# UbiquityRobotics/fiducials

Hardware: NVIDIA H100
Metric: frames/sec 1920x1080 (detect+pose) (higher is better)
Workload: dtype u8/i32 (threshold, contours), f32/f64 (sub-pixel, pose, map)

## Files before the change

### fiducials_b200/csrc/fid_api.cu

```cuda
#include <cuda.h>
#include <cuda_runtime.h>
#include <stdio.h>
#include <stdlib.h>
#include <string.h>

#include <algorithm>
#include <cmath>
#include <vector>

#include "../../include/fiducials_b200.h"
#include "kernels_contour.cuh"
#include "kernels_threshold.cuh"
#include "start_prune_table.h"
#include "kernels_threshold_mma.cuh"
#include "kernels_marker.cuh"
#include "kernels_aruco3.cuh"
#include "params_host.h"

using namespace fid;

#define CK(call)                                                                                       \
    do {                                                                                               \
        cudaError_t e_ = (call);                                                                       \
        if (e_ != cudaSuccess) {                                                                       \
// ... 226 lines not shown
template <class T>
static int halloc(T** p, size_t count) {
    if (cudaMallocHost((void**)p, count * sizeof(T)) != cudaSuccess) {
        cudaGetLastError();
        return FID_ERR_NO_MEMORY;
    }
    return FID_OK;
}

static FrameGeom make_geom(const fid_detector* h, int W, int H, size_t row_stride, size_t frame_stride) {
    FrameGeom g;
    g.W = W;
    g.H = H;
    g.gray_pitch = (W + 31) / 32 * 32;
    g.bgr_row_stride = row_stride;
    g.bgr_frame_stride = frame_stride;
    g.gray_frame_stride = (size_t)g.gray_pitch * H;
    g.halo_tpr = halo_tiles_x(W);
    g.halo_tiles_y = (H + FID_HALO_T - 1) / FID_HALO_T;
    g.halo_scale_stride = halo_plane_words(W, H);
    g.halo_frame_stride = g.halo_scale_stride * h->P.n_scales;
    g.magic_tpr = (uint32_t)((0x100000000ull + (uint64_t)g.halo_tpr - 1) / (uint64_t)g.halo_tpr);
    g.magic_tiles_y = (uint32_t)((0x100000000ull + (uint64_t)g.halo_tiles_y - 1) / (uint64_t)g.halo_tiles_y);
    return g;
}

static int upload_dictionary(fid_detector* h) {
    std::vector<unsigned long long> words;
    pack_dictionary(h->P, &words);
    CK(cudaMemcpy(h->d_dict, words.data(), words.size() * sizeof(unsigned long long), cudaMemcpyHostToDevice));
    return FID_OK;
}

static size_t group_smem(int max_raw) { return (size_t)max_raw * 6 * sizeof(int) + (((size_t)max_raw + 15) & ~(size_t)15) + GROUP_CLOSE_SMEM_WORDS * sizeof(uint32_t); }
static size_t ident_smem(const DevParams& P, int warps) { return (size_t)P.n_markers * 4 * 8 + (size_t)warps * 256 * 4 + (size_t)warps * FID_MAX_WARP_SIDE_SQ; }

typedef CUresult (*EncodeTiledFn)(CUtensorMap*, CUtensorMapDataType, cuuint32_t, void*, const cuuint64_t*, const cuuint64_t*, const cuuint32_t*, const cuuint32_t*, CUtensorMapInterleave,
                                  CUtensorMapSwizzle, CUtensorMapL2promotion, CUtensorMapFloatOOBfill);
static EncodeTiledFn encode_tiled_fn() {
    static EncodeTiledFn fn = nullptr;
    static bool tried = false;
    if (!tried) {
        tried = true;
        void* p = nullptr;
        cudaDriverEntryPointQueryResult q;
        if (cudaGetDriverEntryPoint("cuTensorMapEncodeTiled", &p, cudaEnableDefault, &q) == cudaSuccess && q == cudaDriverEntryPointSuccess) fn = (EncodeTiledFn)p;
        cudaGetLastError();
    }
    return fn;
}
static bool make_bgr_tensor_map(CUtensorMap* tm, const uint8_t* src, int W, int H, int nf, size_t row_stride, size_t frame_stride) {
    EncodeTiledFn fn = encode_tiled_fn();
    if (!fn || (W & 3) || (row_stride & 15) || (frame_stride & 15) || (reinterpret_cast<uintptr_t>(src) & 15) || 3 * W / 4 < TM_BOXW || H < TM_BOXH) return false;
    const cuuint64_t gdim[3] = {(cuuint64_t)(3 * W / 4), (cuuint64_t)H, (cuuint64_t)nf};
    const cuuint64_t gstr[2] = {(cuuint64_t)row_stride, (cuuint64_t)frame_stride};
    const cuuint32_t box[3] = {TM_BOXW, TM_BOXH, 1};
    const cuuint32_t estr[3] = {1, 1, 1};
    return fn(tm, CU_TENSOR_MAP_DATA_TYPE_UINT32, 3, const_cast<uint8_t*>(src), gdim, gstr, box, estr, CU_TENSOR_MAP_INTERLEAVE_NONE, CU_TENSOR_MAP_SWIZZLE_NONE,
              CU_TENSOR_MAP_L2_PROMOTION_L2_128B, CU_TENSOR_MAP_FLOAT_OOB_FILL_NONE) == CUDA_SUCCESS;
}

static int r_max_of(const DevParams& P) {
    int r = 1;
    for (int i = 0; i < P.n_scales; i++) r = std::max(r, P.win[i] / 2);
    return r;
}

static int configure_kernels(fid_detector* h) {
    CK(cudaFuncSetAttribute(k_threshold<true>, cudaFuncAttributeMaxDynamicSharedMemorySize, (int)thresh_smem_bytes(THR_FAST_R)));
    CK(cudaFuncSetAttribute(k_threshold<false>, cudaFuncAttributeMaxDynamicSharedMemorySize, (int)thresh_smem_bytes(FID_MAX_WIN_RADIUS)));
    CK(cudaFuncSetAttribute(k_threshold<true, true>, cudaFuncAttributeMaxDynamicSharedMemorySize, (int)thresh_smem_bytes(THR_FAST_R)));
    CK(cudaFuncSetAttribute(k_threshold<false, true>, cudaFuncAttributeMaxDynamicSharedMemorySize, (int)thresh_smem_bytes(FID_MAX_WIN_RADIUS)));
    CK(cudaFuncSetAttribute(k_threshold_mma<false>, cudaFuncAttributeMaxDynamicSharedMemorySize, (int)TM_SMEM_BYTES));
    CK(cudaFuncSetAttribute(k_threshold_mma<true>, cudaFuncAttributeMaxDynamicSharedMemorySize, (int)TM_SMEM_BYTES));
    for (auto k : {k_sort_group<false>, k_sort_group<true>}) CK(cudaFuncSetAttribute(k, cudaFuncAttributeMaxDynamicSharedMemorySize, (int)group_smem(FID_GROUP_MAX_RAW)));
    for (auto k : {k_identify_retry<false>, k_identify_retry<true>, k_identify_retry<false, true>, k_identify_retry<true, true>, k_identify_retry<false, false, true>,
                   k_identify_retry<true, false, true>, k_identify_retry<false, true, true>, k_identify_retry<true, true, true>})
        CK(cudaFuncSetAttribute(k, cudaFuncAttributeMaxDynamicSharedMemorySize, (int)(kMaxDictMarkers * 4 * 8 + IDENT_WARPS * 256 * 4 + IDENT_WARPS * FID_MAX_WARP_SIDE_SQ)));
    for (auto k : {k_identify_first<false>, k_identify_first<true>, k_identify_first<false, true>, k_identify_first<true, true>, k_identify_first<false, false, true>,
                   k_identify_first<true, false, true>, k_identify_first<false, true, true>, k_identify_first<true, true, true>})
        CK(cudaFuncSetAttribute(k, cudaFuncAttributeMaxDynamicSharedMemorySize, (int)(kMaxDictMarkers * 4 * 8 + IDENT0_WARPS * 256 * 4 + IDENT0_WARPS * FID_MAX_WARP_SIDE_SQ)));
    return FID_OK;
}

static int alloc_slot(fid_detector* h, Slot& s) {
    const size_t F = h->max_batch;
    const int W = h->max_w, H = h->max_h;
    const size_t wpr = (W + 31) / 32, pitch = wpr * 32;
    const int S = FID_MAX_SCALES;
    int rc;
#define A(expr)                  \
    if ((rc = (expr)) != FID_OK) return rc;
    A(dalloc(&s.d_bgr, F * (size_t)W * H * 3));
    A(dalloc(&s.d_gray, F * pitch * H));
    A(dalloc(&s.d_halo, F * (size_t)S * halo_plane_words(W, H)));
    A(dalloc(&s.d_starts, (size_t)h->max_starts));
    A(dalloc(&s.d_chains, (size_t)h->max_chains));
    A(dalloc(&s.d_segs, (size_t)h->max_segs));
    A(dalloc(&s.d_queue[0], (size_t)h->max_queue));
    A(dalloc(&s.d_queue[1], (size_t)h->max_queue));
    A(dalloc(&s.d_points, (size_t)h->max_points));
    A(dalloc(&s.d_counters, 1));
    const size_t R = F * h->max_raw;
    A(dalloc(&s.d_raw, R));
    A(dalloc(&s.d_nraw, F));
    A(dalloc(&s.fs.quads_tmp, R));
    A(dalloc(&s.fs.per_tmp, R));
    A(dalloc(&s.fs.quads, R));
    A(dalloc(&s.fs.per, R));
    A(dalloc(&s.fs.close_bits, R * h->close_wpr));
    A(dalloc(&s.fs.group_id, R));
    A(dalloc(&s.fs.group_members, R));
    A(dalloc(&s.fs.next_in_group, R));
    A(dalloc(&s.fs.group_head, R));
    A(dalloc(&s.fs.group_tail, R));
    A(dalloc(&s.fs.close_count, R));
    A(dalloc(&s.fs.close_idx, R));
    A(dalloc(&s.fs.close_off, R));
    A(dalloc(&s.fs.selected, R));
    A(dalloc(&s.fs.sel_idx, R));
    A(dalloc(&s.fs.raw_of_sorted, R));
    A(dalloc(&s.d_nsel, F));
    A(dalloc(&s.d_nrawc, F));
    A(dalloc(&s.d_cand_id, F * h->max_sel));
    A(dalloc(&s.d_cand_corners, F * h->max_sel * 8));
    A(dalloc(&s.d_cand_raw, F * h->max_sel));
    A(dalloc(&s.d_first_list, F * h->max_sel));
    A(dalloc(&s.d_retry_list, F * h->max_sel));
    const size_t M = F * h->max_markers;
    A(dalloc(&s.d_out_count, F));
    A(dalloc(&s.d_out_ids, M));
    A(dalloc(&s.d_out_corners, M * 8));
    A(dalloc(&s.d_out_tf, M));
    A(halloc(&s.h_out_count, F));
    A(halloc(&s.h_out_ids, M));
    A(halloc(&s.h_out_corners, M * 8));
    A(halloc(&s.h_out_tf, M));
    A(halloc(&s.h_counters, 1));
    A(halloc(&s.h_nsel, F));
    A(halloc(&s.h_nrawc, F));
#undef A
    for (int i = 0; i <= ST_COUNT; i++) CK(cudaEventCreate(&s.ev[i]));
    for (int i = 0; i <= N_WALK_ROUNDS; i++) CK(cudaEventCreate(&s.ev_round[i]));
    CK(cudaEventCreateWithFlags(&s.done, cudaEventDisableTiming));
    CK(cudaEventCreateWithFlags(&s.copied, cudaEventDisableTiming));
// ... 670 lines not shown
    }
    CK(cudaEventRecord(s.ev[ST_APPROX], st));
    {
        ApproxArgs a{};
        a.chains = s.d_chains;
        a.points = s.d_points;
        a.counters = s.d_counters;
        a.raw = s.d_raw;
        a.n_raw = s.d_nraw;
        a.counters_rw = s.d_counters;
        a.max_chains = h->max_chains;
        a.max_raw = h->max_raw;
        a.W = W;
        a.H = H;
        a.poly_accuracy_rate = P.poly_accuracy_rate;
        a.min_corner_dist_rate = P.min_corner_dist_rate;
        launch_prio(k_approx_warp, dim3(h->sm_count * 8), dim3(APPROX_THREADS), 0, st, 3, a);
        launches++;
        launch_prio(k_approx, dim3(h->sm_count * 4), dim3(APPROX_THREADS), 0, st, 3, a);
        launches++;
    }
    CK(cudaEventRecord(s.ev[ST_GROUP], st));
    if (stop_after == ST_APPROX) return FID_OK;
    auto group = [&](int marker_size) {
        GroupArgs a{};
        a.raw = s.d_raw;
        a.n_raw = s.d_nraw;
        a.fs = s.fs;
        a.n_sel = s.d_nsel;
        a.n_raw_clamped = s.d_nrawc;
        a.max_raw = h->max_raw;
        a.close_wpr = h->close_wpr;
        a.max_sel = h->max_sel;
        a.marker_size = marker_size;
        a.border_bits = P.marker_border_bits;
        a.min_marker_dist_rate = (float)P.min_marker_dist_rate;
        a.min_group_dist = (float)P.min_group_dist;
        a.W = W;
        a.H = H;
        a.min_dist_to_border = P.min_dist_to_border;
        a.counters = s.d_counters;
        a.first_list = s.d_first_list;
        static const int group_prof = getenv("FID_GROUP_PROF") ? atoi(getenv("FID_GROUP_PROF")) : 0;
        a.prof = group_prof;
        launch_prio(inv ? k_sort_group<true> : k_sort_group<false>, dim3(nf), dim3(GROUP_THREADS), group_smem(h->max_raw), st, 4, a);
        launches++;
    };
    auto identify = [&](const DevParams& Pd, const unsigned long long* dict) {
        IdentifyArgs a{};
        a.src = d_bgr;
        a.row_stride = g.bgr_row_stride;
        a.frame_stride = g.bgr_frame_stride;
        a.enc = h->enc;
        a.W = g.W;
        a.H = g.H;
        a.fs = s.fs;
        a.n_sel = s.d_nsel;
        a.max_raw = h->max_raw;
        a.max_sel = h->max_sel;
        a.P = Pd;
        a.dict = dict;
        a.cand_id = s.d_cand_id;
        a.cand_corners = s.d_cand_corners;
        a.cand_raw = s.d_cand_raw;
        a.first_list = s.d_first_list;
        a.retry_list = s.d_retry_list;
        a.counters = s.d_counters;
        if (a3) a.pyr = A3Pyramid{s.d_gray, g.gray_frame_stride, s.d_a3_pyr, s.d_raw, ag};
        if (inv) {
            static void (*const first[2][2])(const IdentifyArgs) = {{k_identify_first<false, false, true>, k_identify_first<false, true, true>},
                                                                    {k_identify_first<true, false, true>, k_identify_first<true, true, true>}};
            static void (*const retry[2][2])(const IdentifyArgs) = {{k_identify_retry<false, false, true>, k_identify_retry<false, true, true>},
                                                                    {k_identify_retry<true, false, true>, k_identify_retry<true, true, true>}};
            if (conf) a.cand_conf = s.d_cand_conf;
            launch_prio(first[a3][conf], dim3(h->sm_count * 4), dim3(IDENT0_WARPS * 32), ident_smem(Pd, IDENT0_WARPS), st, 4, a);
            launch_prio(retry[a3][conf], dim3(h->sm_count * 2), dim3(IDENT_WARPS * 32), ident_smem(Pd, IDENT_WARPS), st, 4, a);
        } else if (conf) {
            a.cand_conf = s.d_cand_conf;
// ... 1621 lines not shown
```

### fiducials_b200/csrc/kernels_marker.cuh

```cuda
#pragma once
#include <cuda_runtime.h>

#include "../../include/fiducials_b200.h"
#include "aruco3.cuh"
#include "board_pnp.cuh"
#include "candidate_tree.cuh"
#include "charuco.cuh"
#include "common.cuh"
#include "contour_refine.cuh"
#include "diamond.cuh"
#include "identify.cuh"
#include "ippe.cuh"
#include "marker_refine.cuh"
#include "pnp.cuh"
#include "quad_group.cuh"
#include "subpix.cuh"

namespace fid {


struct FrameScratch {
    QuadF* quads_tmp;
    float* per_tmp;
    QuadF* quads;
    float* per;
    uint32_t* close_bits;
    int* group_id;
    int* group_members;
    int* next_in_group;
    int* group_head;
    int* group_tail;
    int* close_count;
    int* close_idx;
    int* close_off;
    uint8_t* selected;
    int* sel_idx;
    int* raw_of_sorted;
};

struct GroupArgs {
    const RawQuad* raw;
    const unsigned int* n_raw;
    FrameScratch fs;
    int* n_sel;
    int* n_raw_clamped;
    int max_raw, close_wpr, max_sel;
    int marker_size, border_bits;
    float min_marker_dist_rate, min_group_dist;
    int W, H, min_dist_to_border;
    Counters* counters;
    uint32_t* first_list;
    int prof;
};

struct WarpLanes {
    __device__ int lane() const { return threadIdx.x & 31; }
    __device__ int count() const { return 32; }
    __device__ void sync() const { __syncwarp(); }
    __device__ long long sum(long long v) const {
#pragma unroll
        for (int d = 16; d > 0; d >>= 1) v += __shfl_xor_sync(0xffffffffu, v, d);
        return v;
    }
    __device__ int min_i(int v) const {
#pragma unroll
        for (int d = 16; d > 0; d >>= 1) {
            const int o = __shfl_xor_sync(0xffffffffu, v, d);
            v = o < v ? o : v;
        }
        return v;
    }
    __device__ unsigned long long or_u64(unsigned long long v) const {
#pragma unroll
        for (int d = 16; d > 0; d >>= 1) v |= __shfl_xor_sync(0xffffffffu, v, d);
        return v;
    }
    __device__ void hist_add(int* h, int bin) const { atomicAdd(h + bin, 1); }
    __device__ uint32_t ballot(bool p) const { return __ballot_sync(0xffffffffu, p); }
    __device__ int shfl_i(int v, int src) const { return __shfl_sync(0xffffffffu, v, src); }
    __device__ int atomic_add(int* p, int v) const { return atomicAdd(p, v); }
};

#define GROUP_THREADS 1024
#define FID_GROUP_MAX_RAW 4096
#define GROUP_CLOSE_SMEM_WORDS 12288

template <bool INV = false>
__global__ void __launch_bounds__(GROUP_THREADS) k_sort_group(const GroupArgs a) {
    const int f = blockIdx.x;
    const int tid = threadIdx.x;
    int n = (int)a.n_raw[f];
    n = n < a.max_raw ? n : a.max_raw;
    const size_t fo = (size_t)f * a.max_raw;
    const RawQuad* raw = a.raw + fo;
    QuadF* qt = a.fs.quads_tmp + fo;
    float* pt = a.fs.per_tmp + fo;
    QuadF* qs = a.fs.quads + fo;
    float* ps = a.fs.per + fo;
    long long t_[7] = {0, 0, 0, 0, 0, 0, 0};
#define GROUP_TICK(k) if (a.prof && tid == 0 && f == 0) t_[k] = clock64()
    GROUP_TICK(0);
    if (tid == 0) a.n_raw_clamped[f] = n;
    extern __shared__ int sm_group[];
    float* s_f0 = reinterpret_cast<float*>(sm_group);
    float* s_f1 = s_f0 + a.max_raw;
    float* s_f2 = s_f1 + a.max_raw;
    for (int i = tid; i < n; i += GROUP_THREADS) {
        const QuadF q = quad_clockwise(raw[i]);
        qt[i] = q;
        const float p = quad_perimeter(q);
        pt[i] = p;
        s_f0[i] = p;
    }
    __syncthreads();
    for (int i = tid; i < n; i += GROUP_THREADS) {
        const float pi = s_f0[i];
        const uint32_t hi = raw[i].order_hi, lo = raw[i].order_lo;
        int rank = 0;
        for (int j = 0; j < n; j++) {
            const float pj = s_f0[j];
            const bool before = pj > pi || (pj == pi && (raw[j].order_hi < hi || (raw[j].order_hi == hi && raw[j].order_lo < lo)));
            rank += before ? 1 : 0;
        }
        qs[rank] = qt[i];
        ps[rank] = pi;
        a.fs.raw_of_sorted[fo + rank] = i;
    }
    __syncthreads();
    QuadF* s_quads = reinterpret_cast<QuadF*>(s_f2 + a.max_raw);
    const bool quads_in_smem = (size_t)n * sizeof(QuadF) <= (size_t)3 * a.max_raw * sizeof(int);
    for (int i = tid; i < n; i += GROUP_THREADS) {
        const QuadF q = qs[i];
        s_f0[i] = (q.x[0] + q.x[1] + q.x[2] + q.x[3]) * 0.25f;
        s_f1[i] = (q.y[0] + q.y[1] + q.y[2] + q.y[3]) * 0.25f;
        s_f2[i] = ps[i] * a.min_marker_dist_rate;
        if (quads_in_smem) s_quads[i] = q;
    }
    __syncthreads();
    GROUP_TICK(1);
    __shared__ uint32_t row_any[(FID_GROUP_MAX_RAW + 31) / 32], grouped[(FID_GROUP_MAX_RAW + 31) / 32];
    int* sm_group_id = sm_group;
    int* sm_members = sm_group + a.max_raw;
    int* sm_next = sm_group + 3 * a.max_raw;
    int* sm_head = sm_group + 4 * a.max_raw;
    int* sm_tail = sm_group + 5 * a.max_raw;
    uint8_t* sm_selected = reinterpret_cast<uint8_t*>(sm_group + 6 * a.max_raw);
    __shared__ int s_warp_cnt[GROUP_THREADS / 32];
    __shared__ int s_base;
    for (int i = tid; i < (FID_GROUP_MAX_RAW + 31) / 32; i += GROUP_THREADS) row_any[i] = 0;
    __syncthreads();
    const int wpr = (n + 31) >> 5;
    uint32_t* sm_close = reinterpret_cast<uint32_t*>(sm_selected + ((a.max_raw + 15) & ~15));
    const bool close_in_smem = n * wpr <= GROUP_CLOSE_SMEM_WORDS;
    uint32_t* cb = close_in_smem ? sm_close : a.fs.close_bits + fo * a.close_wpr;
    const int cb_pitch = close_in_smem ? wpr : a.close_wpr;
    {
        const int warp = tid >> 5, lane = tid & 31;
        for (int u = warp; u < n * wpr; u += GROUP_THREADS / 32) {
            const int i = u / wpr, w = u - i * wpr;
            const int j0 = w << 5;
            uint32_t bits = 0;
            if (j0 + 31 > i) {
                const int j = j0 + lane;
                bool close = false;
                if (j > i && j < n) {
                    const float thr = s_f2[j];
                    const float dx = s_f0[i] - s_f0[j], dy = s_f1[i] - s_f1[j];
                    const float cd2 = dx * dx + dy * dy;
                    const float lim = thr * 1.01f + 1.0f;
                    if (cd2 <= lim * lim) close = (quads_in_smem ? quad_avg_distance(s_quads[i], s_quads[j]) : quad_avg_distance(qs[i], qs[j])) < thr;
                }
                bits = __ballot_sync(0xffffffffu, close);
            }
            if (lane == 0) {
                cb[(size_t)i * cb_pitch + w] = bits;
                if (bits) atomicOr(&row_any[i >> 5], 1u << (i & 31));
            }
        }
    }
    __syncthreads();
    GROUP_TICK(2);
    __shared__ int s_n_groups, s_total_close, s_members_used;
    __shared__ uint32_t s_row[2][FID_GROUP_MAX_RAW / 32], s_rowmask[2][4];
    if (tid < 32) {
        struct RowPtr {
            const uint32_t* p;
            __device__ uint32_t operator()(int w) const { return p[w]; }
        };
        const int lane = tid;
        int n_groups = 0;
        if (lane == 0) group_pairs_init(n, sm_selected, sm_group_id, sm_next, a.fs.close_count + fo, grouped);
        __syncwarp();
        auto next_row = [&](int i) {
            while (i < n && !((row_any[i >> 5] >> (i & 31)) & 1u)) i++;
            return i;
        };
        if (close_in_smem) {
            if (lane == 0)
                for (int i = next_row(0); i < n; i = next_row(i + 1))
                    group_pairs_row(n, i, RowPtr{sm_close + (size_t)i * wpr}, nullptr, &n_groups, sm_selected, sm_group_id, sm_next, sm_head, sm_tail, grouped);
        } else {
            uint32_t v[3][4];
            int rows[3];
            rows[0] = next_row(0);
            rows[1] = rows[0] < n ? next_row(rows[0] + 1) : n;
            rows[2] = rows[1] < n ? next_row(rows[1] + 1) : n;
#pragma unroll
            for (int r = 0; r < 3; r++)
#pragma unroll
                for (int k = 0; k < 4; k++) v[r][k] = (rows[r] < n && lane + 32 * k < wpr) ? cb[(size_t)rows[r] * cb_pitch + lane + 32 * k] : 0u;
            int buf = 0;
            while (rows[0] < n) {
                const int i = rows[0];
#pragma unroll
                for (int k = 0; k < 4; k++) {
                    if (lane + 32 * k < wpr) s_row[buf][lane + 32 * k] = v[0][k];
                    const uint32_t nz = __ballot_sync(0xffffffffu, v[0][k] != 0u);
                    if (lane == 0) s_rowmask[buf][k] = nz;
                }
                __syncwarp();
                const int inext = rows[2] < n ? next_row(rows[2] + 1) : n;
#pragma unroll
                for (int k = 0; k < 4; k++) {
                    v[0][k] = v[1][k];
                    v[1][k] = v[2][k];
                    v[2][k] = (inext < n && lane + 32 * k < wpr) ? cb[(size_t)inext * cb_pitch + lane + 32 * k] : 0u;
                }
                rows[0] = rows[1];
                rows[1] = rows[2];
                rows[2] = inext;
                if (lane == 0) group_pairs_row(n, i, RowPtr{s_row[buf]}, s_rowmask[buf], &n_groups, sm_selected, sm_group_id, sm_next, sm_head, sm_tail, grouped);
                __syncwarp();
                buf ^= 1;
// ... 70 lines not shown
    int* cand_id;
    float* cand_corners;
    int* cand_raw;
    const uint32_t* first_list;
    uint32_t* retry_list;
    Counters* counters;
    A3Pyramid pyr;
    float* cand_conf;
};

#define IDENT_WARPS 8
#define IDENT0_WARPS 4

__device__ __forceinline__ void identify_write(const IdentifyArgs& a, size_t fo, size_t o, int id, int rot, int used) {
    a.cand_id[o] = id;
    a.cand_raw[o] = a.fs.raw_of_sorted[fo + used];
    const QuadF use = a.fs.quads[fo + used];
    for (int c = 0; c < 4; c++) {
        a.cand_corners[o * 8 + 2 * c] = use.x[(c + 4 - rot) & 3];
        a.cand_corners[o * 8 + 2 * c + 1] = use.y[(c + 4 - rot) & 3];
    }
}

template <bool PYR, bool CONF, bool INV>
__device__ __forceinline__ IdentifyResult identify_attempt(const IdentifyArgs& a, const WarpLanes& L, int f, int level, const QuadF& quad, const unsigned long long* dict,
                                                           uint8_t* img, int* hist) {
    if constexpr (PYR) {
        const float s = a3_level_scale(a.pyr.g, level);
        QuadF q;
        for (int c = 0; c < 4; c++) {
            q.x[c] = quad.x[c] * s;
            q.y[c] = quad.y[c] * s;
        }
        return identify_candidate<CONF, INV>(L, a.pyr.plane(f, level), a.pyr.g.lv[level].W, a.pyr.g.lv[level].H, q, a.P, dict, img, hist);
    } else {
        const FrameImg gray{a.src + (size_t)f * a.frame_stride, a.row_stride, a.enc};
        return identify_candidate<CONF, INV>(L, gray, a.W, a.H, quad, a.P, dict, img, hist);
    }
}
template <bool PYR>
__device__ __forceinline__ int identify_level(const IdentifyArgs& a, size_t fo, int si) {
    if constexpr (PYR)
        return a3_level_for(a.pyr.g, a.pyr.raw[fo + a.fs.raw_of_sorted[fo + si]].n_contour);
    else
        return 0;
}

template <bool PYR, bool CONF = false, bool INV = false>
__global__ void __launch_bounds__(IDENT0_WARPS * 32) k_identify_first(const IdentifyArgs a) {
    extern __shared__ unsigned long long sm_dict[];
    const unsigned int n_first = a.counters->n_first;
    if (blockIdx.x * IDENT0_WARPS >= n_first) return;
    const int n_words = a.P.n_markers * 4;
    for (int i = threadIdx.x; i < n_words; i += blockDim.x) sm_dict[i] = __ldg(a.dict + i);
    const int warp = threadIdx.x >> 5, lane = threadIdx.x & 31;
    int* hist = reinterpret_cast<int*>(sm_dict + n_words) + warp * 256;
    uint8_t* img = reinterpret_cast<uint8_t*>(reinterpret_cast<int*>(sm_dict + n_words) + IDENT0_WARPS * 256) + warp * (FID_MAX_WARP_SIDE_SQ);
    __syncthreads();
    WarpLanes L;
    for (unsigned int i = blockIdx.x * IDENT0_WARPS + warp; i < n_first; i += gridDim.x * IDENT0_WARPS) {
        const uint32_t rec = a.first_list[i];
        const int f = (int)(rec >> 16), k = (int)(rec & 0xFFFFu);
        const size_t fo = (size_t)f * a.max_raw, o = (size_t)f * a.max_sel + k;
        const int si = a.fs.sel_idx[fo + k];
        const IdentifyResult r = identify_attempt<PYR, CONF, INV>(a, L, f, identify_level<PYR>(a, fo, si), a.fs.quads[fo + si], sm_dict, img, hist);
        __syncwarp();
        if (lane == 0) {
            if (r.id >= 0) {
                identify_write(a, fo, o, r.id, r.rotation, si);
                if constexpr (CONF) a.cand_conf[o] = marker_confidence(hist, a.P, sm_dict[r.id * 4 + r.rotation]);
            } else if (a.fs.close_count[fo + si] > 0) {
                a.cand_id[o] = -2;
                a.retry_list[atomicAdd(&a.counters->n_retry, 1u)] = rec;
            } else {
                a.cand_id[o] = -1;
            }
        }
        if constexpr (CONF) __syncwarp();
    }
}

template <bool PYR, bool CONF = false, bool INV = false>
__global__ void __launch_bounds__(IDENT_WARPS * 32) k_identify_retry(const IdentifyArgs a) {
    extern __shared__ unsigned long long sm_dict[];
    __shared__ int s_best;
    __shared__ int s_id[IDENT_WARPS], s_rot[IDENT_WARPS], s_att[IDENT_WARPS];
    const unsigned int n_retry = a.counters->n_retry;
    if (blockIdx.x >= n_retry) return;
    const int n_words = a.P.n_markers * 4;
    for (int i = threadIdx.x; i < n_words; i += blockDim.x) sm_dict[i] = __ldg(a.dict + i);
    const int warp = threadIdx.x >> 5, lane = threadIdx.x & 31;
    int* hist = reinterpret_cast<int*>(sm_dict + n_words) + warp * 256;
    uint8_t* img = reinterpret_cast<uint8_t*>(reinterpret_cast<int*>(sm_dict + n_words) + IDENT_WARPS * 256) + warp * (FID_MAX_WARP_SIDE_SQ);
    WarpLanes L;
    for (unsigned int i = blockIdx.x; i < n_retry; i += gridDim.x) {
        const uint32_t rec = a.retry_list[i];
        const int f = (int)(rec >> 16), k = (int)(rec & 0xFFFFu);
        const size_t fo = (size_t)f * a.max_raw, o = (size_t)f * a.max_sel + k;
        __syncthreads();
        if (threadIdx.x == 0) s_best = 0x7fffffff;
        if (lane == 0) s_att[warp] = 0x7fffffff;
        __syncthreads();
        const int si = a.fs.sel_idx[fo + k];
        const int level = identify_level<PYR>(a, fo, si);
        const int nc = a.fs.close_count[fo + si], co = a.fs.close_off[fo + si];
        for (int t = 1 + warp; t <= nc; t += IDENT_WARPS) {
            if (t > *reinterpret_cast<volatile int*>(&s_best)) break;
            const QuadF quad = a.fs.quads[fo + a.fs.close_idx[fo + co + t - 1]];
            const IdentifyResult r = identify_attempt<PYR, CONF, INV>(a, L, f, level, quad, sm_dict, img, hist);
            __syncwarp();
            if (r.id >= 0) {
                if (lane == 0) {
                    s_id[warp] = r.id;
                    s_rot[warp] = r.rotation;
                    s_att[warp] = t;
                    atomicMin(&s_best, t);
// ... 1186 lines not shown
```

### fiducials_b200/csrc/identify.cuh

```cuda
#pragma once
#include "common.cuh"
#include "quad_group.cuh"

namespace fid {

struct SerialLanes {
    FID_HD int lane() const { return 0; }
    FID_HD int count() const { return 1; }
    FID_HD void sync() const {}
    FID_HD long long sum(long long v) const { return v; }
    FID_HD int min_i(int v) const { return v; }
    FID_HD unsigned long long or_u64(unsigned long long v) const { return v; }
    FID_HD void hist_add(int* h, int bin) const { h[bin]++; }
    FID_HD uint32_t ballot(bool p) const { return p ? 1u : 0u; }
    FID_HD int shfl_i(int v, int) const { return v; }
    FID_HD int atomic_add(int* p, int v) const {
        const int old = *p;
        *p += v;
        return old;
    }
};

FID_HD bool perspective_transform(const QuadF& q, double size_minus_1, double M[9]) {
    double A[8][8], B[8];
    const double dx[4] = {0.0, size_minus_1, size_minus_1, 0.0};
    const double dy[4] = {0.0, 0.0, size_minus_1, size_minus_1};
    for (int i = 0; i < 4; i++) {
        const double sx = q.x[i], sy = q.y[i];
        A[i][0] = A[i + 4][3] = sx;
        A[i][1] = A[i + 4][4] = sy;
        A[i][2] = A[i + 4][5] = 1.0;
        A[i][3] = A[i][4] = A[i][5] = A[i + 4][0] = A[i + 4][1] = A[i + 4][2] = 0.0;
        A[i][6] = -sx * dx[i];
        A[i][7] = -sy * dx[i];
        A[i + 4][6] = -sx * dy[i];
        A[i + 4][7] = -sy * dy[i];
        B[i] = dx[i];
        B[i + 4] = dy[i];
    }
    for (int i = 0; i < 8; i++) {
        int k = i;
        for (int j = i + 1; j < 8; j++)
            if (fabs(A[j][i]) > fabs(A[k][i])) k = j;
        if (fabs(A[k][i]) < 2.220446049250313e-16 * 100) return false;
        if (k != i) {
            for (int j = i; j < 8; j++) {
                const double t = A[i][j];
                A[i][j] = A[k][j];
// ... 55 lines not shown
    double fy = (Y0 + Mi[3] * x) * w;
    fx = fx < -2147483648.0 ? -2147483648.0 : (fx > 2147483647.0 ? 2147483647.0 : fx);
    fy = fy < -2147483648.0 ? -2147483648.0 : (fy > 2147483647.0 ? 2147483647.0 : fy);
    const int sx = round_half_even_to_int(fx), sy = round_half_even_to_int(fy);
    if ((unsigned)sx < (unsigned)W && (unsigned)sy < (unsigned)H) return gray.at(sx, sy);
    return 0;
}

FID_HD int otsu_threshold(const int* h, int total) {
    double mu = 0.0;
    const double scale = 1.0 / (double)total;
    for (int i = 0; i < 256; i++) mu += i * (double)h[i];
    mu *= scale;
    double mu1 = 0.0, q1 = 0.0, max_sigma = 0.0;
    int max_val = 0;
    for (int i = 0; i < 256; i++) {
        const double p_i = h[i] * scale;
        mu1 *= q1;
        q1 += p_i;
        const double q2 = 1.0 - q1;
        const double lo = q1 < q2 ? q1 : q2, hi = q1 < q2 ? q2 : q1;
        if (lo < 1.1920928955078125e-07 || hi > 1.0 - 1.1920928955078125e-07) continue;
        mu1 = (mu1 + i * p_i) / q1;
        const double mu2 = (mu - q1 * mu1) / q2;
        const double sigma = q1 * q2 * (mu1 - mu2) * (mu1 - mu2);
        if (sigma > max_sigma) {
            max_sigma = sigma;
            max_val = i;
        }
    }
    return max_val;
}

struct IdentifyResult {
    int id;
    int rotation;
    bool inverted;
};

struct CellBits {
    unsigned long long lo, hi;
    bool ok;
    FID_HD int at(int c) const { return (int)(((c < 64 ? lo >> c : hi >> (c - 64))) & 1ull); }
};

template <bool CONF = false, class Lanes, class Img>
FID_HD CellBits extract_bits(const Lanes& L, const Img& gray, int W, int H, const QuadF& quad, const DevParams& P, uint8_t* img, int* hist) {
    CellBits out = {0ull, 0ull, false};
    const int cells = P.marker_size + 2 * P.marker_border_bits;
    const int cell = P.px_per_cell;
    const int S = cells * cell;
    const int margin = (int)(P.ignored_margin_per_cell * cell);
    double M[9], Mi[9];
    if (!perspective_transform(quad, (double)(S - 1), M)) return out;
    if (!invert3x3(M, Mi)) return out;
    for (int i = L.lane(); i < 256; i += L.count()) hist[i] = 0;
    L.sync();
    const int half = cell / 2;
    long long s1 = 0, s2 = 0;
    for (int p = L.lane(); p < S * S; p += L.count()) {
        const int y = p / S, x = p - y * S;
        const int v = warp_nearest_sample(gray, W, H, Mi, x, y);
        img[p] = (uint8_t)v;
        L.hist_add(hist, v);
        if (x >= half && x < S - half && y >= half && y < S - half) {
            s1 += v;
            s2 += v * v;
        }
    }
    s1 = L.sum(s1);
    s2 = L.sum(s2);
    L.sync();
    const int inner = (S - 2 * half) * (S - 2 * half);
    const double scale = 1.0 / (double)inner;
    const double mean = (double)s1 * scale;
    double var = (double)s2 * scale - mean * mean;
    var = var > 0.0 ? var : 0.0;
    const double stddev = sqrt(var);
    unsigned long long bits_lo = 0, bits_hi = 0;
    if (stddev < P.min_otsu_stddev) {
        if (mean > 127.0) bits_lo = bits_hi = ~0ull;
        if constexpr (CONF) {
            const int win = cell - 2 * margin;
            L.sync();
            for (int c = L.lane(); c < cells * cells; c += L.count()) hist[c] = mean > 127.0 ? win * win : 0;
            L.sync();
        }
    } else {
        const int t = otsu_threshold(hist, S * S);
        const int win = cell - 2 * margin;
        if constexpr (CONF) L.sync();
        unsigned long long mine = 0, mine_hi = 0;
        for (int c = L.lane(); c < cells * cells; c += L.count()) {
            const int cy = c / cells, cx = c - cy * cells;
            int nz = 0;
            for (int yy = 0; yy < win; yy++)
                for (int xx = 0; xx < win; xx++) nz += img[(cy * cell + margin + yy) * S + cx * cell + margin + xx] > t ? 1 : 0;
            if constexpr (CONF) hist[c] = nz;
            if (nz > (win * win) / 2) {
                if (c < 64)
                    mine |= 1ull << c;
                else
                    mine_hi |= 1ull << (c - 64);
            }
        }
        bits_lo = L.or_u64(mine);
        bits_hi = cells * cells > 64 ? L.or_u64(mine_hi) : 0ull;
        if constexpr (CONF) L.sync();
    }
    out.lo = bits_lo;
    out.hi = bits_hi;
    out.ok = true;
    return out;
}

FID_HD unsigned long long inner_code(const CellBits& b, const DevParams& P) {
    const int cells = P.marker_size + 2 * P.marker_border_bits;
    const int bb = P.marker_border_bits, ms = P.marker_size;
    unsigned long long cand = 0;
    int k = 0, cur = 0, nbits = 0, byte_i = 0;
    const int total = ms * ms;
    for (int y = 0; y < ms; y++)
// ... 4 lines not shown
            if (nbits == 8 || k == total) {
                cand |= (unsigned long long)cur << (8 * byte_i);
                byte_i++;
                cur = 0;
                nbits = 0;
            }
        }
    return cand;
}

FID_HD float marker_confidence(const int* cnt, const DevParams& P, unsigned long long word) {
    const int bb = P.marker_border_bits, ms = P.marker_size, cells = ms + 2 * bb;
    const int margin = (int)(P.ignored_margin_per_cell * P.px_per_cell);
    const int win = P.px_per_cell - 2 * margin;
    const float area = (float)(win * win);
    const int total = ms * ms, last_byte = (total - 1) >> 3, last_bits = total & 7 ? total & 7 : 8;
    double sum = 0.0;
    for (int y = 0; y < cells; y++)
        for (int x = 0; x < cells; x++) {
            const float ratio = (float)cnt[y * cells + x] / area;
            bool one = false;
            if (y >= bb && y < cells - bb && x >= bb && x < cells - bb) {
                const int k = (y - bb) * ms + x - bb, byte = k >> 3;
                const int nb = byte == last_byte ? last_bits : 8;
                one = (word >> (8 * byte + nb - 1 - (k & 7))) & 1ull;
            }
            sum += one ? 1.0f - ratio : ratio;
        }
    return 1.0f - (float)sum / (float)(cells * cells);
}

template <bool CONF = false, bool INV = false, class Lanes, class Img>
FID_HD IdentifyResult identify_candidate(const Lanes& L, const Img& gray, int W, int H, const QuadF& quad, const DevParams& P, const unsigned long long* dict, uint8_t* img,
                                         int* hist) {
    IdentifyResult res = {-1, 0, false};
    CellBits bits = extract_bits<CONF>(L, gray, W, H, quad, P, img, hist);
    if (!bits.ok) return res;
    const int cells = P.marker_size + 2 * P.marker_border_bits;
    const int bb = P.marker_border_bits, ms = P.marker_size;
    int border_errors = 0;
    for (int y = 0; y < cells; y++)
        for (int x = 0; x < cells; x++) {
            const bool in_border = y < bb || y >= cells - bb || x < bb || x >= cells - bb;
            if (in_border && bits.at(y * cells + x)) border_errors++;
        }
    if constexpr (INV) {
        const int inv_errors = cells * cells - ms * ms - border_errors;
        if (inv_errors < border_errors) {
            border_errors = inv_errors;
            bits.lo = ~bits.lo;
            bits.hi = ~bits.hi;
            res.inverted = true;
            if constexpr (CONF) {
                const int margin = (int)(P.ignored_margin_per_cell * P.px_per_cell);
                const int win = P.px_per_cell - 2 * margin;
                for (int c = L.lane(); c < cells * cells; c += L.count()) hist[c] = win * win - hist[c];
                L.sync();
            }
        }
    }
    const int max_border = (int)((double)(ms * ms) * P.max_err_border_rate);
    if (border_errors > max_border) return res;
    const unsigned long long cand = inner_code(bits, P);
    const int max_corr = (int)((double)P.max_correction_bits * P.error_correction_rate);
    int first = 0x7fffffff;
    for (int m = L.lane(); m < P.n_markers; m += L.count()) {
        int best = ms * ms + 1, rot = -1;
        for (int r = 0; r < 4; r++) {
            const unsigned long long d = dict[m * 4 + r] ^ cand;
// ... 21 lines not shown
```

Measured before the change: 10860.

## Shrink sort_group block, store close bits triangular, plan shared memory per frame

Reduces k_sort_group from 1024 to 256 threads with a 48KB dynamic shared memory budget and launch bounds targeting four blocks per SM. Shared memory is now laid out per frame from the actual candidate count, with a fallback to global buffers for each part that does not fit. The close-pair bitmask is stored as an upper-triangular matrix so larger candidate counts fit in shared memory. The rank sort also processes four elements per thread and caches order keys in shared memory. The aim is more resident blocks, fewer global accesses and cheaper ranking. The cost is fewer threads per frame and an extra global path for large n.

```diff
diff --git a/fiducials_b200/csrc/fid_api.cu b/fiducials_b200/csrc/fid_api.cu
--- a/fiducials_b200/csrc/fid_api.cu
+++ b/fiducials_b200/csrc/fid_api.cu
@@ -282,7 +282,6 @@
     return FID_OK;
 }
 
-static size_t group_smem(int max_raw) { return (size_t)max_raw * 6 * sizeof(int) + (((size_t)max_raw + 15) & ~(size_t)15) + GROUP_CLOSE_SMEM_WORDS * sizeof(uint32_t); }
 static size_t ident_smem(const DevParams& P, int warps) { return (size_t)P.n_markers * 4 * 8 + (size_t)warps * 256 * 4 + (size_t)warps * FID_MAX_WARP_SIDE_SQ; }
 
 typedef CUresult (*EncodeTiledFn)(CUtensorMap*, CUtensorMapDataType, cuuint32_t, void*, const cuuint64_t*, const cuuint64_t*, const cuuint32_t*, const cuuint32_t*, CUtensorMapInterleave,
@@ -323,7 +322,7 @@
     CK(cudaFuncSetAttribute(k_threshold<false, true>, cudaFuncAttributeMaxDynamicSharedMemorySize, (int)thresh_smem_bytes(FID_MAX_WIN_RADIUS)));
     CK(cudaFuncSetAttribute(k_threshold_mma<false>, cudaFuncAttributeMaxDynamicSharedMemorySize, (int)TM_SMEM_BYTES));
     CK(cudaFuncSetAttribute(k_threshold_mma<true>, cudaFuncAttributeMaxDynamicSharedMemorySize, (int)TM_SMEM_BYTES));
-    for (auto k : {k_sort_group<false>, k_sort_group<true>}) CK(cudaFuncSetAttribute(k, cudaFuncAttributeMaxDynamicSharedMemorySize, (int)group_smem(FID_GROUP_MAX_RAW)));
+    for (auto k : {k_sort_group<false>, k_sort_group<true>}) CK(cudaFuncSetAttribute(k, cudaFuncAttributeMaxDynamicSharedMemorySize, GROUP_SMEM_BYTES));
     for (auto k : {k_identify_retry<false>, k_identify_retry<true>, k_identify_retry<false, true>, k_identify_retry<true, true>, k_identify_retry<false, false, true>,
                    k_identify_retry<true, false, true>, k_identify_retry<false, true, true>, k_identify_retry<true, true, true>})
         CK(cudaFuncSetAttribute(k, cudaFuncAttributeMaxDynamicSharedMemorySize, (int)(kMaxDictMarkers * 4 * 8 + IDENT_WARPS * 256 * 4 + IDENT_WARPS * FID_MAX_WARP_SIDE_SQ)));
@@ -360,7 +359,7 @@
     A(dalloc(&s.fs.per, R));
     A(dalloc(&s.fs.close_bits, R * h->close_wpr));
     A(dalloc(&s.fs.group_id, R));
-    A(dalloc(&s.fs.group_members, R));
+    A(dalloc(&s.fs.group_members, 2 * R));
     A(dalloc(&s.fs.next_in_group, R));
     A(dalloc(&s.fs.group_head, R));
     A(dalloc(&s.fs.group_tail, R));
@@ -1097,6 +1096,7 @@
         a.max_raw = h->max_raw;
         a.close_wpr = h->close_wpr;
         a.max_sel = h->max_sel;
+        a.smem_bytes = GROUP_SMEM_BYTES;
         a.marker_size = marker_size;
         a.border_bits = P.marker_border_bits;
         a.min_marker_dist_rate = (float)P.min_marker_dist_rate;
@@ -1108,7 +1108,7 @@
         a.first_list = s.d_first_list;
         static const int group_prof = getenv("FID_GROUP_PROF") ? atoi(getenv("FID_GROUP_PROF")) : 0;
         a.prof = group_prof;
-        launch_prio(inv ? k_sort_group<true> : k_sort_group<false>, dim3(nf), dim3(GROUP_THREADS), group_smem(h->max_raw), st, 4, a);
+        launch_prio(inv ? k_sort_group<true> : k_sort_group<false>, dim3(nf), dim3(GROUP_THREADS), GROUP_SMEM_BYTES, st, 4, a);
         launches++;
     };
     auto identify = [&](const DevParams& Pd, const unsigned long long* dict) {
diff --git a/fiducials_b200/csrc/kernels_marker.cuh b/fiducials_b200/csrc/kernels_marker.cuh
--- a/fiducials_b200/csrc/kernels_marker.cuh
+++ b/fiducials_b200/csrc/kernels_marker.cuh
@@ -45,6 +45,7 @@
     int* n_sel;
     int* n_raw_clamped;
     int max_raw, close_wpr, max_sel;
+    int smem_bytes;
     int marker_size, border_bits;
     float min_marker_dist_rate, min_group_dist;
     int W, H, min_dist_to_border;
@@ -81,12 +82,36 @@
     __device__ int atomic_add(int* p, int v) const { return atomicAdd(p, v); }
 };
 
-#define GROUP_THREADS 1024
+#define GROUP_THREADS 256
 #define FID_GROUP_MAX_RAW 4096
-#define GROUP_CLOSE_SMEM_WORDS 12288
+#define GROUP_SMEM_BYTES 49152
+#define GROUP_RANK_ILP 4
+
+FID_HD int group_tri_row(int i, int wpr) {
+    const int b = i >> 5;
+    return 32 * (b * wpr - b * (b - 1) / 2) + (i - 32 * b) * (wpr - b);
+}
+
+struct GroupSmemPlan {
+    int scratch, close, quads;
+};
+FID_HD size_t group_align16(size_t b) { return (b + 15) & ~(size_t)15; }
+FID_HD GroupSmemPlan group_smem_plan(int n, int smem_bytes) {
+    GroupSmemPlan p{-1, -1, -1};
+    size_t used = 0;
+    const size_t parts[3] = {group_align16((size_t)n * (6 * sizeof(int) + 1)), group_align16((size_t)group_tri_row(n, (n + 31) >> 5) * sizeof(uint32_t)),
+                             (size_t)n * sizeof(QuadF)};
+    int* offs[3] = {&p.scratch, &p.close, &p.quads};
+    for (int k = 0; k < 3; k++)
+        if (used + parts[k] <= (size_t)smem_bytes) {
+            *offs[k] = (int)used;
+            used += parts[k];
+        }
+    return p;
+}
 
 template <bool INV = false>
-__global__ void __launch_bounds__(GROUP_THREADS) k_sort_group(const GroupArgs a) {
+__global__ void __launch_bounds__(GROUP_THREADS, 4) k_sort_group(const GroupArgs a) {
     const int f = blockIdx.x;
     const int tid = threadIdx.x;
     int n = (int)a.n_raw[f];
@@ -101,34 +126,77 @@
 #define GROUP_TICK(k) if (a.prof && tid == 0 && f == 0) t_[k] = clock64()
     GROUP_TICK(0);
     if (tid == 0) a.n_raw_clamped[f] = n;
-    extern __shared__ int sm_group[];
-    float* s_f0 = reinterpret_cast<float*>(sm_group);
-    float* s_f1 = s_f0 + a.max_raw;
-    float* s_f2 = s_f1 + a.max_raw;
+    extern __shared__ __align__(16) unsigned char sm_group[];
+    const GroupSmemPlan plan = group_smem_plan(n, a.smem_bytes);
+    int *sm_group_id, *sm_members, *sm_next, *sm_head, *sm_tail;
+    uint8_t* sm_selected;
+    if (plan.scratch >= 0) {
+        sm_group_id = reinterpret_cast<int*>(sm_group + plan.scratch);
+        sm_members = sm_group_id + n;
+        sm_next = sm_members + 2 * n;
+        sm_head = sm_next + n;
+        sm_tail = sm_head + n;
+        sm_selected = reinterpret_cast<uint8_t*>(sm_tail + n);
+    } else {
+        sm_group_id = a.fs.group_id + fo;
+        sm_members = a.fs.group_members + 2 * fo;
+        sm_next = a.fs.next_in_group + fo;
+        sm_head = a.fs.group_head + fo;
+        sm_tail = a.fs.group_tail + fo;
+        sm_selected = a.fs.selected + fo;
+    }
+    float* s_f0 = reinterpret_cast<float*>(sm_group_id);
+    float* s_f1 = reinterpret_cast<float*>(sm_members);
+    float* s_f2 = s_f1 + n;
     for (int i = tid; i < n; i += GROUP_THREADS) {
         const QuadF q = quad_clockwise(raw[i]);
         qt[i] = q;
         const float p = quad_perimeter(q);
         pt[i] = p;
         s_f0[i] = p;
-    }
-    __syncthreads();
-    for (int i = tid; i < n; i += GROUP_THREADS) {
-        const float pi = s_f0[i];
-        const uint32_t hi = raw[i].order_hi, lo = raw[i].order_lo;
-        int rank = 0;
-        for (int j = 0; j < n; j++) {
-            const float pj = s_f0[j];
-            const bool before = pj > pi || (pj == pi && (raw[j].order_hi < hi || (raw[j].order_hi == hi && raw[j].order_lo < lo)));
-            rank += before ? 1 : 0;
-        }
-        qs[rank] = qt[i];
-        ps[rank] = pi;
-        a.fs.raw_of_sorted[fo + rank] = i;
-    }
-    __syncthreads();
-    QuadF* s_quads = reinterpret_cast<QuadF*>(s_f2 + a.max_raw);
-    const bool quads_in_smem = (size_t)n * sizeof(QuadF) <= (size_t)3 * a.max_raw * sizeof(int);
+        reinterpret_cast<uint32_t*>(s_f1)[i] = raw[i].order_hi;
+        reinterpret_cast<uint32_t*>(s_f2)[i] = raw[i].order_lo;
+    }
+    __syncthreads();
+    {
+        const uint32_t* s_hi = reinterpret_cast<const uint32_t*>(s_f1);
+        const uint32_t* s_lo = reinterpret_cast<const uint32_t*>(s_f2);
+        for (int i0 = tid; i0 < n; i0 += GROUP_THREADS * GROUP_RANK_ILP) {
+            float pi[GROUP_RANK_ILP];
+            uint32_t hi[GROUP_RANK_ILP], lo[GROUP_RANK_ILP];
+            int rank[GROUP_RANK_ILP];
+#pragma unroll
+            for (int r = 0; r < GROUP_RANK_ILP; r++) {
+                const int i = i0 + r * GROUP_THREADS;
+                const bool in = i < n;
+                pi[r] = in ? s_f0[i] : 0.f;
+                hi[r] = in ? s_hi[i] : 0u;
+                lo[r] = in ? s_lo[i] : 0u;
+                rank[r] = 0;
+            }
+            for (int j = 0; j < n; j++) {
+                const float pj = s_f0[j];
+                const uint32_t hj = s_hi[j], lj = s_lo[j];
+#pragma unroll
+                for (int r = 0; r < GROUP_RANK_ILP; r++) {
+                    const bool before = pj > pi[r] || (pj == pi[r] && (hj < hi[r] || (hj == hi[r] && lj < lo[r])));
+                    rank[r] += before ? 1 : 0;
+                }
+            }
+#pragma unroll
+            for (int r = 0; r < GROUP_RANK_ILP; r++) {
+                const int i = i0 + r * GROUP_THREADS;
+                if (i < n) {
+                    qs[rank[r]] = qt[i];
+                    ps[rank[r]] = pi[r];
+                    a.fs.raw_of_sorted[fo + rank[r]] = i;
+                }
+            }
+        }
+    }
+    __syncthreads();
+    QuadF* s_quads = reinterpret_cast<QuadF*>(sm_group + plan.quads);
+    const bool quads_in_smem = plan.quads >= 0;
     for (int i = tid; i < n; i += GROUP_THREADS) {
         const QuadF q = qs[i];
         s_f0[i] = (q.x[0] + q.x[1] + q.x[2] + q.x[3]) * 0.25f;
@@ -139,29 +207,23 @@
     __syncthreads();
     GROUP_TICK(1);
     __shared__ uint32_t row_any[(FID_GROUP_MAX_RAW + 31) / 32], grouped[(FID_GROUP_MAX_RAW + 31) / 32];
-    int* sm_group_id = sm_group;
-    int* sm_members = sm_group + a.max_raw;
-    int* sm_next = sm_group + 3 * a.max_raw;
-    int* sm_head = sm_group + 4 * a.max_raw;
-    int* sm_tail = sm_group + 5 * a.max_raw;
-    uint8_t* sm_selected = reinterpret_cast<uint8_t*>(sm_group + 6 * a.max_raw);
     __shared__ int s_warp_cnt[GROUP_THREADS / 32];
     __shared__ int s_base;
     for (int i = tid; i < (FID_GROUP_MAX_RAW + 31) / 32; i += GROUP_THREADS) row_any[i] = 0;
     __syncthreads();
     const int wpr = (n + 31) >> 5;
-    uint32_t* sm_close = reinterpret_cast<uint32_t*>(sm_selected + ((a.max_raw + 15) & ~15));
-    const bool close_in_smem = n * wpr <= GROUP_CLOSE_SMEM_WORDS;
-    uint32_t* cb = close_in_smem ? sm_close : a.fs.close_bits + fo * a.close_wpr;
-    const int cb_pitch = close_in_smem ? wpr : a.close_wpr;
+    uint32_t* sm_close = reinterpret_cast<uint32_t*>(sm_group + plan.close);
+    const bool close_in_smem = plan.close >= 0;
+    uint32_t* cb = a.fs.close_bits + fo * a.close_wpr;
+    const int cb_pitch = a.close_wpr;
+    auto close_row = [&](int i) { return close_in_smem ? sm_close + group_tri_row(i, wpr) - (i >> 5) : cb + (size_t)i * cb_pitch; };
     {
         const int warp = tid >> 5, lane = tid & 31;
-        for (int u = warp; u < n * wpr; u += GROUP_THREADS / 32) {
-            const int i = u / wpr, w = u - i * wpr;
-            const int j0 = w << 5;
-            uint32_t bits = 0;
-            if (j0 + 31 > i) {
-                const int j = j0 + lane;
+        for (int i = warp; i < n; i += GROUP_THREADS / 32) {
+            uint32_t* row = close_row(i);
+            uint32_t any = 0;
+            for (int w = i >> 5; w < wpr; w++) {
+                const int j = (w << 5) + lane;
                 bool close = false;
                 if (j > i && j < n) {
                     const float thr = s_f2[j];
@@ -170,12 +232,11 @@
                     const float lim = thr * 1.01f + 1.0f;
                     if (cd2 <= lim * lim) close = (quads_in_smem ? quad_avg_distance(s_quads[i], s_quads[j]) : quad_avg_distance(qs[i], qs[j])) < thr;
                 }
-                bits = __ballot_sync(0xffffffffu, close);
-            }
-            if (lane == 0) {
-                cb[(size_t)i * cb_pitch + w] = bits;
-                if (bits) atomicOr(&row_any[i >> 5], 1u << (i & 31));
-            }
+                const uint32_t bits = __ballot_sync(0xffffffffu, close);
+                if (lane == 0) row[w] = bits;
+                any |= bits;
+            }
+            if (lane == 0 && any) atomicOr(&row_any[i >> 5], 1u << (i & 31));
         }
     }
     __syncthreads();
@@ -198,7 +259,7 @@
         if (close_in_smem) {
             if (lane == 0)
                 for (int i = next_row(0); i < n; i = next_row(i + 1))
-                    group_pairs_row(n, i, RowPtr{sm_close + (size_t)i * wpr}, nullptr, &n_groups, sm_selected, sm_group_id, sm_next, sm_head, sm_tail, grouped);
+                    group_pairs_row(n, i, RowPtr{close_row(i)}, nullptr, &n_groups, sm_selected, sm_group_id, sm_next, sm_head, sm_tail, grouped);
         } else {
             uint32_t v[3][4];
             int rows[3];
```

After: 11080, median of 6. 2.0% higher.

## Parallelize Otsu threshold across warp lanes with exactness fallback

Applied to the files above, without the earlier changes.

Replaces the serial per-warp Otsu threshold scan with a lane-parallel version. Lane 0 builds the cumulative class probabilities, the reciprocals are computed in parallel, and an FMA-corrected recurrence reproduces the serial mean. The between-class variance is then evaluated by all lanes and reduced with a shuffle argmax. Scratch space is taken from the unused tail of the warp's sample buffer, and the code falls back to the serial routine if any lane detects a rounding mismatch. Min-blocks-per-SM hints are also added to both identify kernels, which may cap registers and cause spills.

```diff
diff --git a/fiducials_b200/csrc/identify.cuh b/fiducials_b200/csrc/identify.cuh
--- a/fiducials_b200/csrc/identify.cuh
+++ b/fiducials_b200/csrc/identify.cuh
@@ -14,6 +14,7 @@
     FID_HD void hist_add(int* h, int bin) const { h[bin]++; }
     FID_HD uint32_t ballot(bool p) const { return p ? 1u : 0u; }
     FID_HD int shfl_i(int v, int) const { return v; }
+    FID_HD int argmax_first(double, int i) const { return i; }
     FID_HD int atomic_add(int* p, int v) const {
         const int old = *p;
         *p += v;
@@ -135,6 +136,79 @@
     return max_val;
 }
 
+FID_HD double fma_rn(double a, double b, double c) {
+#if defined(__CUDA_ARCH__)
+    return __fma_rn(a, b, c);
+#else
+    return fma(a, b, c);
+#endif
+}
+
+FID_HD bool otsu_bin_trivial(double q1) {
+    const double q2 = 1.0 - q1;
+    const double lo = q1 < q2 ? q1 : q2, hi = q1 < q2 ? q2 : q1;
+    return lo < 1.1920928955078125e-07 || hi > 1.0 - 1.1920928955078125e-07;
+}
+
+#define FID_OTSU_SCRATCH_BYTES (512 * 8)
+
+template <class Lanes>
+FID_HD int otsu_threshold_lanes(const Lanes& L, const int* h, int total, double* s) {
+    double* q1s = s;
+    double* rm = s + 256;
+    const double scale = 1.0 / (double)total;
+    long long m = 0;
+    for (int i = L.lane(); i < 256; i += L.count()) m += (long long)i * h[i];
+    const double mu = (double)L.sum(m) * scale;
+    int i0 = 256, i1 = -1;
+    if (L.lane() == 0) {
+        double q1 = 0.0;
+        for (int i = 0; i < 256; i++) {
+            q1 += h[i] * scale;
+            q1s[i] = q1;
+            if (!otsu_bin_trivial(q1)) {
+                i0 = i0 < i ? i0 : i;
+                i1 = i;
+            }
+        }
+    }
+    i0 = L.shfl_i(i0, 0);
+    i1 = L.shfl_i(i1, 0);
+    L.sync();
+    for (int i = i0 + L.lane(); i <= i1; i += L.count()) rm[i] = 1.0 / q1s[i];
+    L.sync();
+    if (L.lane() == 0) {
+        double mu1 = 0.0, qp = i0 > 0 ? q1s[i0 - 1] : 0.0;
+        for (int i = i0; i <= i1; i++) {
+            const double q = q1s[i], r = rm[i];
+            const double x = mu1 * qp + i * (h[i] * scale);
+            const double y0 = x * r;
+            mu1 = fma_rn(fma_rn(-q, y0, x), r, y0);
+            rm[i] = mu1;
+            qp = q;
+        }
+    }
+    L.sync();
+    bool exact = true;
+    double best = 0.0;
+    int best_i = 0;
+    for (int i = i0 + L.lane(); i <= i1; i += L.count()) {
+        const double q1 = q1s[i], q2 = 1.0 - q1, mu1 = rm[i];
+        const double x = (i > i0 ? rm[i - 1] * q1s[i - 1] : 0.0) + i * (h[i] * scale);
+        exact = exact && x / q1 == mu1;
+        const double mu2 = (mu - q1 * mu1) / q2;
+        const double sigma = q1 * q2 * (mu1 - mu2) * (mu1 - mu2);
+        if (sigma > best) {
+            best = sigma;
+            best_i = i;
+        }
+    }
+    const bool any_inexact = L.ballot(!exact) != 0u;
+    L.sync();
+    if (any_inexact) return otsu_threshold(h, total);
+    return L.argmax_first(best, best_i);
+}
+
 struct IdentifyResult {
     int id;
     int rotation;
@@ -148,7 +222,8 @@
 };
 
 template <bool CONF = false, class Lanes, class Img>
-FID_HD CellBits extract_bits(const Lanes& L, const Img& gray, int W, int H, const QuadF& quad, const DevParams& P, uint8_t* img, int* hist) {
+FID_HD CellBits extract_bits(const Lanes& L, const Img& gray, int W, int H, const QuadF& quad, const DevParams& P, uint8_t* img, int* hist,
+                             int img_bytes = 0) {
     CellBits out = {0ull, 0ull, false};
     const int cells = P.marker_size + 2 * P.marker_border_bits;
     const int cell = P.px_per_cell;
@@ -190,7 +265,9 @@
             L.sync();
         }
     } else {
-        const int t = otsu_threshold(hist, S * S);
+        const int otsu_at = (S * S + 7) & ~7;
+        const int t = otsu_at + FID_OTSU_SCRATCH_BYTES <= img_bytes ? otsu_threshold_lanes(L, hist, S * S, reinterpret_cast<double*>(img + otsu_at))
+                                                                     : otsu_threshold(hist, S * S);
         const int win = cell - 2 * margin;
         if constexpr (CONF) L.sync();
         unsigned long long mine = 0, mine_hi = 0;
@@ -261,9 +338,9 @@
 
 template <bool CONF = false, bool INV = false, class Lanes, class Img>
 FID_HD IdentifyResult identify_candidate(const Lanes& L, const Img& gray, int W, int H, const QuadF& quad, const DevParams& P, const unsigned long long* dict, uint8_t* img,
-                                         int* hist) {
+                                         int* hist, int img_bytes = 0) {
     IdentifyResult res = {-1, 0, false};
-    CellBits bits = extract_bits<CONF>(L, gray, W, H, quad, P, img, hist);
+    CellBits bits = extract_bits<CONF>(L, gray, W, H, quad, P, img, hist, img_bytes);
     if (!bits.ok) return res;
     const int cells = P.marker_size + 2 * P.marker_border_bits;
     const int bb = P.marker_border_bits, ms = P.marker_size;
diff --git a/fiducials_b200/csrc/kernels_marker.cuh b/fiducials_b200/csrc/kernels_marker.cuh
--- a/fiducials_b200/csrc/kernels_marker.cuh
+++ b/fiducials_b200/csrc/kernels_marker.cuh
@@ -78,6 +78,18 @@
     __device__ void hist_add(int* h, int bin) const { atomicAdd(h + bin, 1); }
     __device__ uint32_t ballot(bool p) const { return __ballot_sync(0xffffffffu, p); }
     __device__ int shfl_i(int v, int src) const { return __shfl_sync(0xffffffffu, v, src); }
+    __device__ int argmax_first(double v, int i) const {
+#pragma unroll
+        for (int d = 16; d > 0; d >>= 1) {
+            const double ov = __shfl_xor_sync(0xffffffffu, v, d);
+            const int oi = __shfl_xor_sync(0xffffffffu, i, d);
+            if (ov > v || (ov == v && oi < i)) {
+                v = ov;
+                i = oi;
+            }
+        }
+        return i;
+    }
     __device__ int atomic_add(int* p, int v) const { return atomicAdd(p, v); }
 };
 
@@ -335,10 +347,10 @@
             q.x[c] = quad.x[c] * s;
             q.y[c] = quad.y[c] * s;
         }
-        return identify_candidate<CONF, INV>(L, a.pyr.plane(f, level), a.pyr.g.lv[level].W, a.pyr.g.lv[level].H, q, a.P, dict, img, hist);
+        return identify_candidate<CONF, INV>(L, a.pyr.plane(f, level), a.pyr.g.lv[level].W, a.pyr.g.lv[level].H, q, a.P, dict, img, hist, FID_MAX_WARP_SIDE_SQ);
     } else {
         const FrameImg gray{a.src + (size_t)f * a.frame_stride, a.row_stride, a.enc};
-        return identify_candidate<CONF, INV>(L, gray, a.W, a.H, quad, a.P, dict, img, hist);
+        return identify_candidate<CONF, INV>(L, gray, a.W, a.H, quad, a.P, dict, img, hist, FID_MAX_WARP_SIDE_SQ);
     }
 }
 template <bool PYR>
@@ -350,7 +362,7 @@
 }
 
 template <bool PYR, bool CONF = false, bool INV = false>
-__global__ void __launch_bounds__(IDENT0_WARPS * 32) k_identify_first(const IdentifyArgs a) {
+__global__ void __launch_bounds__(IDENT0_WARPS * 32, 8) k_identify_first(const IdentifyArgs a) {
     extern __shared__ unsigned long long sm_dict[];
     const unsigned int n_first = a.counters->n_first;
     if (blockIdx.x * IDENT0_WARPS >= n_first) return;
@@ -384,7 +396,7 @@
 }
 
 template <bool PYR, bool CONF = false, bool INV = false>
-__global__ void __launch_bounds__(IDENT_WARPS * 32) k_identify_retry(const IdentifyArgs a) {
+__global__ void __launch_bounds__(IDENT_WARPS * 32, 4) k_identify_retry(const IdentifyArgs a) {
     extern __shared__ unsigned long long sm_dict[];
     __shared__ int s_best;
     __shared__ int s_id[IDENT_WARPS], s_rot[IDENT_WARPS], s_att[IDENT_WARPS];
```

Measured after the change: 10850 before, 10860 after (median of 6 runs). Within noise of the previous version (+0.1%).
